# valette/FROG

Hardware: AMD Instinct MI355X
Metric: registration iterations/sec (linear+deformable) (higher is better)
Workload: dtype f32

## Files before the change

frog_amd/_abi.py:

```python
import ctypes as C
import os

_HERE = os.path.dirname(os.path.abspath(__file__))
LIB_DIR = os.path.join(_HERE, "lib")



def usable_cpus():
    import math
    n = len(os.sched_getaffinity(0)) if hasattr(os, "sched_getaffinity") else (os.cpu_count() or 1)

    def quota(d):
        try:
            with open(os.path.join(d, "cpu.max")) as fh:
                q, p = fh.read().split()[:2]
            return None if q == "max" else float(q) / float(p)
        except (OSError, ValueError):
            pass
        try:
            with open(os.path.join(d, "cpu.cfs_quota_us")) as fh:
                q = float(fh.read())
            with open(os.path.join(d, "cpu.cfs_period_us")) as fh:
                p = float(fh.read())
            return q / p if q > 0 and p > 0 else None
# ... 278 lines not shown
    "frog_deformable_phase_b": (C.c_int, [C.c_void_p]),
    "frog_deformable_phase_c": (C.c_int, [C.c_void_p, c_double_p]),
    "frog_get_stream": (C.c_int, [C.c_void_p, C.POINTER(C.c_void_p), C.POINTER(C.c_int)]),
    "frog_comm_unpack_slab": (C.c_int, [C.c_void_p, C.c_void_p, C.c_uint64, C.c_uint32, C.POINTER(C.c_uint64), C.c_uint32]),
    "frog_comm_mode": (C.c_int, [C.c_void_p, C.c_int]),
    "frog_create_seconds": (C.c_int, [C.c_void_p, c_double_p, C.POINTER(C.c_int)]),
    "frog_lattice_reallocations": (C.c_int, [C.c_void_p, C.POINTER(C.c_int)]),
    "frog_transform_points_slab": (C.c_int, [C.c_void_p, C.c_int, C.c_int, C.c_void_p, C.c_uint64, C.c_uint32]),
    "frog_comm_unpack_slab_step": (C.c_int, [C.c_void_p, C.c_void_p, C.c_uint64, C.c_uint32, C.POINTER(C.c_uint64), C.c_uint32, C.c_uint32]),
    "frog_step_finish": (C.c_int, [C.c_void_p, C.POINTER(C.c_double)]),
    "frog_step_speculate": (C.c_int, [C.c_void_p]),
    "frog_cull_stats": (C.c_int, [C.c_void_p, C.POINTER(C.c_uint64), C.POINTER(C.c_uint64), C.POINTER(C.c_uint64)]),
    "frog_cull_stats_linear": (C.c_int, [C.c_void_p, C.POINTER(C.c_uint64), C.POINTER(C.c_uint64), C.POINTER(C.c_uint64)]),
    "frog_test_stray_points": (C.c_int, [C.c_void_p, C.POINTER(C.c_uint64)]),
    "frog_test_cull_ranges": (C.c_int, [C.c_void_p, C.POINTER(C.c_uint64), C.POINTER(C.c_uint64)]),
    "frog_test_em_refit": (C.c_int, [C.c_void_p, C.c_int]),
    "frog_test_inlier_probability": (C.c_int, [C.c_int, c_float_p, c_float_p, C.c_size_t, c_float_p, c_float_p]),
    "frog_test_inlier_weight_pair": (C.c_int, [C.c_int, c_float_p, c_float_p, C.c_float, c_float_p, C.c_size_t, c_float_p,
                                              C.POINTER(C.c_ubyte)]),
    "frog_test_bspline_weights": (C.c_int, [C.c_int, C.c_void_p, C.c_size_t, C.c_void_p]),
    "frog_profile_enable": (C.c_int, [C.c_void_p, C.c_int]),
    "frog_profile_read": (C.c_int, [C.c_void_p, C.POINTER(FrogKernelTime), C.c_int]),
}

HOST_SYMBOLS = {
    "frog_pairs_read": (C.c_void_p, [C.c_char_p, C.POINTER(C.c_int)]),
    "frog_pairs_write": (C.c_int, [C.c_void_p, C.c_char_p]),
    "frog_pairs_free": (None, [C.c_void_p]),
    "frog_pairs_model": (None, [C.c_void_p, C.POINTER(FrogModel)]),
    "frog_pairs_num_pairs": (C.c_uint64, [C.c_void_p]),
# ... 109 lines not shown
```

frog_amd/csrc/device/ctx.h:

```cpp
#pragma once

#include <hip/hip_runtime.h>

#include <cstdint>
#include <cstdio>
#include <cstring>
#include <string>
#include <memory>
#include <vector>

#include "../../../include/frog_hip.h"
#include "dev_buf.h"
#include "switches.h"

namespace frog {

extern thread_local std::string g_last_error;

inline int fail(int code, const std::string &msg)
{
    g_last_error = msg;
    return code;
}

// ... 258 lines not shown
    frog::DevBuf<uint32_t> rc_group_len;
    frog::DevBuf<uint64_t> rc_group_size, rc_group_ptr;
    frog::DevBuf<uint32_t> rc_ent;
    frog::DevBuf<double> rc_wt;

    bool exact_weights = false;
    float fast_theta() const { return sw.weight_general ? __builtin_nanf("") : opt.inlier_threshold - 1e-4f; }
    bool cull_enabled = true;
    bool cull_need_build = true;
    bool cull_linear = true;
    uint64_t cull_lin_builds = 0;
    frog::DevBuf<unsigned long long> lin_listed;
    frog::DevBuf<uint32_t> act_recs32;
    frog::DevBuf<frog::LinkRec> act_recs;
    frog::DevBuf<uint32_t> act_cnt;
    bool pos_b_stale = true;
    frog::DevBuf<float4> pos_b;
    frog::DevBuf<frog::P3> pos2_snap;
    frog::DevBuf<float> cut_now, cut_list;
    frog::DevBuf<uint32_t> disp_part;
    uint32_t disp_n = 0;
    uint32_t disp_own_n = 0;
    bool disp_others = false;
    frog::DevBuf<uint32_t> cull_state;
    frog::DevBuf<float> disp_allow;
    frog::DevBuf<float4> retired_arena;
    size_t retired_used = 0;
    bool coeff_zero = false;
    bool build_in_sweep = false;
    bool cull_check_due = true;
// ... 21 lines not shown
```

frog_amd/csrc/device/frog_hip.hip:

```cpp

#include "ctx.h"
#include <hip/hip_ext.h>
#include "prep.h"
#include "k_links.hip.h"
#include "k_stats.hip.h"
#include "k_grid.hip.h"
#include "k_comm.hip.h"
#include "k_cull.hip.h"
#include "k_ransac.hip.h"
#include "k_reforder.hip.h"
#include "k_refchain.hip.h"
#include "similarity.h"

#include <atomic>
#include <chrono>
#include <cmath>
#include <cstdlib>
#include <random>
#include <limits>
#include <new>

namespace frog {
thread_local std::string g_last_error;
constexpr int BOUNDS_BLOCKS = 256;
// ... 90 lines not shown
}

static SweepArgs sweep_args(frog_ctx *ctx, uint32_t sub)
{
    SweepArgs a;
    a.sub = sub;
    a.n_groups = ctx->n_groups;
    for (uint32_t g = 0; g <= ctx->n_groups; g++) a.group_begin[g] = ctx->group_begin[g];
    a.tiles = ctx->tiles.p; a.recs = ctx->rec_format.narrow ? (const void *)ctx->recs32.p : (const void *)ctx->recs.p; a.pos2 = ctx->pos2.p; a.emd = ctx->emd.p; a.emf = ctx->emf.p; a.em = ctx->em.p;
    a.rec2_last = (uint32_t)(ctx->L_recs / 2 - 1);
    a.img_bits = ctx->rec_format.img_bits; a.lds_images = sweep_lds_images(ctx); a.poff = ctx->d_poff.p; a.point_last = (uint32_t)(ctx->P ? ctx->P - 1 : 0);
    a.n_tiles = ctx->n_tiles; a.threshold = ctx->opt.inlier_threshold;
    a.band = ctx->exact_weights ? __builtin_inff() : THRESHOLD_BAND;
    a.tile_partial = ctx->tile_partial.p; a.tile_counts = ctx->tile_counts.p; a.group_sums = ctx->group_sums.p;
    a.own_pt_begin = ctx->own_pt_begin; a.own_points = ctx->own_pt_end - ctx->own_pt_begin;
    a.act_recs = nullptr; a.act_cnt = nullptr; a.cull_state = nullptr;
    a.cut_list = nullptr; a.build_recs = nullptr; a.build_cnt = nullptr;
    a.point_sums = ctx->point_sums.p; a.tile_order = ctx->tile_order.p; a.tiles_bo = ctx->tiles_bo.p;
    return a;
}

static bool cull_active(const frog_ctx *ctx)
{
    return ctx->cull_enabled && ctx->deformable && ctx->opt.inlier_threshold >= 1e-3f && ctx->n_tiles > 0;
}

static bool cull_active_linear(const frog_ctx *ctx)
{
    return ctx->cull_enabled && ctx->cull_linear && !ctx->exact_weights && !ctx->deformable && ctx->n_tiles > 0 && ctx->n_sub == 1;
}

static bool sweep_builds_list(const frog_ctx *ctx) { return ctx->rec_format.narrow != 0; }
// ... 2 lines not shown
{
    return ctx->fused_sweep && !build;
}

template <int MODE>
static void launch_sweep(frog_ctx *ctx, uint32_t sub, hipStream_t s, hipEvent_t ea = nullptr, hipEvent_t eb = nullptr,
                         bool use_list = false, bool build_list = false)
{
    uint32_t widest = 0;
    for (uint32_t g = 0; g < ctx->n_groups; g++) widest = std::max(widest, ctx->group_begin[g + 1] - ctx->group_begin[g]);
    if (ctx->n_tiles == 0) return;
    SweepArgs args = sweep_args(ctx, sub);
    if (use_list) {
        args.act_recs = ctx->rec_format.narrow ? (const void *)ctx->act_recs32.p : (const void *)ctx->act_recs.p;
        args.act_cnt = ctx->act_cnt.p;
        args.cull_state = ctx->cull_state.p;
    }
    const dim3 grid(sweep_blocks(ctx)), block(256);
    const size_t lds = (size_t)args.lds_images * (sizeof(EmDerived) + sizeof(uint32_t) + sizeof(float));
    if constexpr (MODE == SWEEP_LINEAR) {
        if (build_list && sweep_builds_list(ctx)) {
            args.act_recs = nullptr; args.act_cnt = nullptr;
            args.cut_list = ctx->cut_list.p; args.build_recs = ctx->act_recs32.p; args.build_cnt = ctx->act_cnt.p;
            hipExtLaunchKernelGGL((sweep_kernel<SWEEP_LINEAR, true, false, true>), grid, block, lds, s, ea, eb, 0, args);
            return;
        }
    }
    if constexpr (MODE == SWEEP_DEFORMABLE) {
        const bool build = build_list && sweep_builds_list(ctx);
        if (build) {
            args.act_recs = nullptr; args.act_cnt = nullptr;
            args.cut_list = ctx->cut_list.p; args.build_recs = ctx->act_recs32.p; args.build_cnt = ctx->act_cnt.p;
        }
        if (sweep_fused_now(ctx, build)) {
            const dim3 fgrid(ctx->n_order_blocks), fblock(512);
            const size_t flds = lds * N_XCD;
            if (ctx->rec_format.narrow) hipExtLaunchKernelGGL((sweep_kernel<SWEEP_DEFORMABLE, true, false, false, true>), fgrid, fblock, flds, s, ea, eb, 0, args);
            else hipExtLaunchKernelGGL((sweep_kernel<SWEEP_DEFORMABLE, true, true, false, true>), fgrid, fblock, flds, s, ea, eb, 0, args);
            return;
        }
        if (build) {
            hipExtLaunchKernelGGL((sweep_kernel<SWEEP_DEFORMABLE, true, false, true>), grid, block, lds, s, ea, eb, 0, args);
            return;
        }
    }
    if (ctx->rec_format.narrow)
        hipExtLaunchKernelGGL((sweep_kernel<MODE, true, false>), grid, block, lds, s, ea, eb, 0, args);
// ... 940 lines not shown
    if (o->n_fixed_images) {
        const uint32_t nf = (uint32_t)o->n_fixed_images;
        if (o->n_fixed_images < 0 || nf >= m->n_images) return fail(FROG_E_INVALID, "n_fixed_images must leave at least one moving image");
        if (image_begin != 0 || image_end != m->n_images)
            return fail(FROG_E_INVALID, "n_fixed_images needs the whole group in one context");
        frog_options o2 = *o;
        o2.n_fixed_images = 0;
        frog_ctx *moving = nullptr, *fixed = nullptr;
        int rc = frog_create(m, &o2, device, nf, m->n_images, &moving);
        if (rc) return rc;
        frog_options o3 = o2;
        o3.max_levels_hint = 0;
        rc = frog_create(m, &o3, device, 0, nf, &fixed);
        if (rc) { frog_destroy(moving); return rc; }
        fixed->cull_enabled = false;
        fixed->act_recs32.release(); fixed->act_recs.release(); fixed->act_cnt.release(); fixed->pos2_snap.release();
        rc = frog_set_stream(fixed, moving->stream);
        if (rc) { frog_destroy(fixed); frog_destroy(moving); return rc; }
        moving->helper = fixed;
        moving->nf = nf;
        moving->opt.n_fixed_images = o->n_fixed_images;
        *out = moving;
        return FROG_OK;
    }
    frog_ctx *c = new (std::nothrow) frog_ctx;
    if (!c) return fail(FROG_E_NOMEM, "out of host memory");
    c->sw = read_switches(MAX_SUBPASS);
    c->device = device;
    c->opt = *o;
    c->ib = image_begin; c->ie = image_end;
    if (const int rc = create_stages(c, m)) {
// ... 604 lines not shown
        return fail(FROG_E_STATE, "context owns a sub-range of images: use frog_bounds_local + all-reduce + frog_deformable_setup_bounds");
    double mn[3], mx[3];
    int rc = frog_bounds_local(ctx, mn, mx);
    if (rc) return rc;
    return frog_deformable_setup_bounds(ctx, level, mn, mx, out);
}

static int cull_allocate_buffers(frog_ctx *ctx);

static int cull_allocate(frog_ctx *ctx)
{
    if (ctx->act_cnt.p || !ctx->cull_enabled) return FROG_OK;
    const int rc = cull_allocate_buffers(ctx);
    if (rc == FROG_OK) return rc;
    (void)hipGetLastError();
    ctx->act_recs32.release(); ctx->act_recs.release(); ctx->act_cnt.release(); ctx->pos2_snap.release();
    ctx->cut_list.release(); ctx->disp_part.release(); ctx->cull_state.release(); ctx->disp_allow.release();
    ctx->cull_enabled = false;
    ctx->fused_sweep = ctx->fused_sweep && ctx->sw.fused == 1;
    return FROG_OK;
}

static int cull_allocate_buffers(frog_ctx *ctx)
{
    hipStream_t s = ctx->stream;
    if (ctx->rec_format.narrow) {
        FROG_HIP_CHECK(ctx->act_recs32.alloc(ctx->L_recs));
        FROG_HIP_CHECK(hipMemsetAsync(ctx->act_recs32.p, 0, ctx->act_recs32.bytes(), s));
    } else {
        FROG_HIP_CHECK(ctx->act_recs.alloc(ctx->L_recs));
        FROG_HIP_CHECK(hipMemsetAsync(ctx->act_recs.p, 0, ctx->act_recs.bytes(), s));
    }
    FROG_HIP_CHECK(ctx->act_cnt.alloc(std::max<size_t>(1, (size_t)ctx->n_tiles * ctx->n_groups)));
    FROG_HIP_CHECK(ctx->pos2_snap.alloc(ctx->P));
    FROG_HIP_CHECK(ctx->cut_list.alloc(ctx->nI));
    {
        uint32_t blocks = 0;
        for (uint32_t i = 0; i < ctx->nI; i++) blocks += div_up(ctx->poff[i + 1] - ctx->poff[i], CULL_BLOCK_POINTS);
        FROG_HIP_CHECK(ctx->disp_part.alloc(std::max<size_t>(blocks, (size_t)ctx->P + ctx->P / SCATTER_CHUNK + 16)));
    }
    FROG_HIP_CHECK(ctx->cull_state.alloc(2));
    FROG_HIP_CHECK(hipMemsetAsync(ctx->cull_state.p, 0, ctx->cull_state.bytes(), s));
    FROG_HIP_CHECK(ctx->disp_allow.alloc(1));
    FROG_HIP_CHECK(hipMemsetAsync(ctx->disp_allow.p, 0xFF, sizeof(float), s));
    ctx->cull_need_build = true;
    return FROG_OK;
}

static int cull_prepare(frog_ctx *ctx)
{
    hipStream_t s = ctx->stream;
    const uint32_t nI = ctx->nI;
    int rc = cull_allocate(ctx);
    if (rc) return rc;
    if (!ctx->cull_enabled) return FROG_OK;
    if (ctx->cull_need_build) {
        cull_list_cutoff_kernel<<<div_up(nI, 64), 64, 0, s>>>(ctx->cut_now.p, nI, ctx->deformable ? ctx->sw.cull_scale : ctx->sw.cull_lin_scale,
                                                              ctx->deformable ? ctx->sw.cull_pad : ctx->sw.cull_lin_pad, ctx->cut_list.p);
        FROG_HIP_CHECK(hipMemcpyAsync(ctx->pos2_snap.p, ctx->pos2.p, ctx->P * sizeof(P3), hipMemcpyDeviceToDevice, s));
        ctx->build_in_sweep = sweep_builds_list(ctx) && !ctx->sw.cull_build_pass;
        if (!ctx->build_in_sweep) {
            const SweepArgs args = sweep_args(ctx, 0);
            const dim3 grid(sweep_blocks(ctx), ctx->n_sub);
            if (ctx->rec_format.narrow)
                cull_build_kernel<false><<<grid, 256, 0, s>>>(args, ctx->cut_list.p, ctx->act_recs32.p, ctx->act_cnt.p);
            else
                cull_build_kernel<true><<<grid, 256, 0, s>>>(args, ctx->cut_list.p, ctx->act_recs.p, ctx->act_cnt.p);
            FROG_HIP_CHECK(hipGetLastError());
        }
        ctx->cull_need_build = false;
        if (ctx->deformable) ctx->cull_builds++; else ctx->cull_lin_builds++;
        ctx->disp_n = 0;
        ctx->disp_own_n = 0;
        ctx->disp_current = true;
        ctx->disp_others = true;
        ctx->cull_check_due = true;
    }
    const bool measured = ctx->disp_current && ((ctx->whole_group() && !ctx->xyz2_exported) || ctx->disp_others);
    if (!measured) {
        uint32_t max_pts = 1;
        for (uint32_t i = 0; i < nI; i++) max_pts = std::max(max_pts, ctx->poff[i + 1] - ctx->poff[i]);
        const dim3 grid(div_up(max_pts, CULL_BLOCK_POINTS), nI);
// ... 606 lines not shown
    CTX_GUARD(ctx);
    if (!ranges || !with_election) return fail(FROG_E_INVALID, "null output");
    *ranges = 0; *with_election = 0;
    if (ctx->cull_builds && ctx->act_cnt.n) {
        std::vector<uint32_t> h(ctx->act_cnt.n);
        FROG_HIP_CHECK(hipMemcpyAsync(h.data(), ctx->act_cnt.p, ctx->act_cnt.bytes(), hipMemcpyDeviceToHost, ctx->stream));
        FROG_HIP_CHECK(hipStreamSynchronize(ctx->stream));
        for (uint32_t v : h) {
            if (v & ~CULL_DUP_BIT) (*ranges)++;
            if (v & CULL_DUP_BIT) (*with_election)++;
        }
    }
    return FROG_OK;
}

int frog_test_stray_points(frog_ctx *ctx, uint64_t *n)
{
    CTX_GUARD(ctx);
    { const int rc_ = join_setup(ctx); if (rc_) return rc_; }
    if (!n) return fail(FROG_E_INVALID, "null output");
    unsigned int v = 0;
    FROG_HIP_CHECK(hipMemcpyAsync(&v, ctx->stray.p + 2, sizeof v, hipMemcpyDeviceToHost, ctx->stream));
    FROG_HIP_CHECK(hipStreamSynchronize(ctx->stream));
    *n = v;
    return FROG_OK;
}

int frog_test_em_refit(frog_ctx *ctx, int term_by_term)
{
    CTX_GUARD(ctx);
// ... 199 lines not shown
```

frog_amd/csrc/device/k_cull.hip.h:

```cpp
#pragma once

#include "ctx.h"
#include "k_links.hip.h"
#include "k_stats.hip.h"

namespace frog {

__device__ inline double mixture_probability(double d, double c1, double c2, double ratio)
{
    const double eps = 1e-10, c = 0.797884560802865;
    const double a = d / (c1 + eps), b = d / (c2 + eps);
    const double x1 = ratio * c * a * a * exp(-0.5 * a * a) / (c1 + eps);
    const double x2 = (1.0 - ratio) * c * b * b * exp(-0.5 * b * b) / (c2 + eps);
    return x1 / (x1 + x2 + eps);
}

__device__ inline float cull_cutoff_of(const float4 e, float threshold);

__global__ void cull_cutoff_kernel(const float4 *em, uint32_t n_images, float threshold, float *cut_now)
{
    const uint32_t i = blockIdx.x * blockDim.x + threadIdx.x;
    if (i >= n_images) return;
    cut_now[i] = cull_cutoff_of(em[i], threshold);
}
// ... 43 lines not shown
                out = (float)hi;
            }
        }
        if (out < __builtin_inff()) out = out * 1.000001f + 1e-6f;
    }
    return out;
}

__global__ void cull_list_cutoff_kernel(const float *cut_now, uint32_t n_images, float scale, float pad, float *cut_list)
{
    const uint32_t i = blockIdx.x * blockDim.x + threadIdx.x;
    if (i < n_images) cut_list[i] = scale * cut_now[i] + pad;
}

template <bool WIDE>
__global__ __launch_bounds__(256) void cull_build_kernel(const SweepArgs a, const float *cut_list, void *act_recs, uint32_t *act_cnt)
{
    const int wave = threadIdx.x >> 6, lane = threadIdx.x & 63;
    const uint32_t xcd = blockIdx.x % N_XCD;
    const uint32_t grp = blockIdx.y * N_XCD + xcd;
    const uint32_t t = (blockIdx.x / N_XCD) * 4 + wave;
    if (t >= a.n_tiles) return;
    const Tile &tl = a.tiles[t];
    const uint32_t pt_begin = tl.pt_begin, image = tl.image;
    const uint32_t rec_lo = tl.rec_begin + tl.group_off[grp], rec_n = tl.group_cnt[grp];
    const uint32_t g_first = a.group_begin[grp];
    const float cutA = cut_list[image];
    using Rec = std::conditional_t<WIDE, unsigned long long, unsigned int>;
    const Rec *src = reinterpret_cast<const Rec *>(a.recs);
    Rec *dst = reinterpret_cast<Rec *>(act_recs);
    auto phys = [&](uint32_t k) { return (size_t)rec_lo + (k / REC_CHUNK) * REC_CHUNK + (k % 64u) * 2u + (k % REC_CHUNK) / 64u; };
    __shared__ uint32_t last_step_s[4][TILE_POINTS];
    uint32_t *last_step = last_step_s[wave];
    for (int k = lane; k < TILE_POINTS; k += 64) last_step[k] = 0xFFFFFFFFu;
    __builtin_amdgcn_fence(__ATOMIC_RELEASE, "wavefront");
    __builtin_amdgcn_wave_barrier();
    bool dup = false;
    uint32_t base = 0;
    constexpr int UNROLL = 4;
    for (uint32_t k0 = 0; k0 < rec_n; k0 += 64 * UNROLL) {
        Rec rq[UNROLL];
        bool have[UNROLL];
        #pragma unroll
        for (int u = 0; u < UNROLL; u++) {
            const uint32_t k = k0 + 64 * u + lane;
            have[u] = k < rec_n;
            rq[u] = have[u] ? src[phys(k)] : (Rec)0;
        }
        P3 pa[UNROLL], pb[UNROLL];
        uint32_t imgB[UNROLL];
        #pragma unroll
        for (int u = 0; u < UNROLL; u++) {
// ... 4 lines not shown
                pb_index = (uint32_t)(rq[u] >> 32);
            } else {
                imgB[u] = g_first + __builtin_amdgcn_ubfe((uint32_t)rq[u], 8u, a.img_bits);
                pb_index = a.poff[imgB[u]] + ((uint32_t)rq[u] >> (8u + a.img_bits));
            }
            pa[u] = a.pos2[pt_begin + ia];
            pb[u] = a.pos2[min(pb_index, a.point_last)];
        }
        #pragma unroll
        for (int u = 0; u < UNROLL; u++) {
            const float dx = pb[u].x - pa[u].x, dy = pb[u].y - pa[u].y, dz = pb[u].z - pa[u].z;
            const float d2 = dx * dx + dy * dy + dz * dz;
            const float cut = have[u] ? fminf(cutA, cut_list[imgB[u]]) : 0.f;
            const bool keep = have[u] && !(d2 >= cut * cut);
            const unsigned long long m = __ballot(keep);
            if (keep) {
                const uint32_t to = base + (uint32_t)__popcll(m & ((1ull << lane) - 1ull));
                dst[phys(to)] = rq[u];
                dup |= atomicExch(&last_step[(uint32_t)rq[u] & 0xFFu], to >> 6) == (to >> 6);
            }
            base += (uint32_t)__popcll(m);
        }
    }
    const bool any_dup = __ballot(dup) != 0ull;
    if (lane == 0) act_cnt[(size_t)t * a.n_groups + grp] = base | (any_dup ? CULL_DUP_BIT : 0u);
    const uint32_t cap = (rec_n + REC_CHUNK - 1) / REC_CHUNK * REC_CHUNK;
    const uint32_t reach = (((base + 63u) / 64u + BODY_STEPS - 1u) / BODY_STEPS * BODY_STEPS + PT_AHEAD) * 64u;
    for (uint32_t k = base + lane; k < min(cap, reach); k += 64) dst[phys(k)] = (Rec)0;
}

constexpr int CULL_BLOCK_POINTS = 2048;

__global__ __launch_bounds__(256) void cull_disp_kernel(const P3 *pos2, const P3 *snap, const uint32_t *poff, uint32_t *disp_part)
{
    __shared__ uint32_t sh[4];
    const uint32_t img = blockIdx.y;
    const uint32_t p0 = poff[img] + blockIdx.x * CULL_BLOCK_POINTS, pe = poff[img + 1];
    const uint32_t p1 = min(p0 + (uint32_t)CULL_BLOCK_POINTS, pe);
    uint32_t m = 0;
// ... 117 lines not shown
```

frog_amd/csrc/device/k_links.hip.h:

```cpp
#pragma once

#include "ctx.h"

#include <type_traits>

namespace frog {

enum { SWEEP_LINEAR = 0, SWEEP_DEFORMABLE = 1, SWEEP_COUNT = 2 };
constexpr int CHUNK_RING = 3, CHUNK_AHEAD = 2;
constexpr int PT_RING = 3, PT_AHEAD = 2;
constexpr int BODY_STEPS = 6;
static_assert(BODY_STEPS == 2 * CHUNK_RING && BODY_STEPS % PT_RING == 0 && PT_AHEAD < PT_RING && CHUNK_AHEAD < CHUNK_RING
              && 2 * CHUNK_AHEAD >= PT_AHEAD + 2, "ring periods must divide the unrolled body; a gather needs its record");
constexpr int EMD_LDS_IMAGES = 256;
constexpr uint32_t CULL_DUP_BIT = 0x80000000u;
constexpr int OWNER_WORDS = TILE_POINTS / 2;
static_assert((OWNER_WORDS & (OWNER_WORDS - 1)) == 0, "the election word of a point is its index masked");
static_assert(EMD_LDS_IMAGES == 1 << 8, "prep.h admits narrow records for img_bits <= 8 only");
constexpr int LINEAR_SUMS = 18;

struct SweepArgs {
    const Tile *tiles;
    const void *recs;
    const uint32_t *poff;
    uint32_t img_bits;
    uint32_t lds_images;
    uint32_t point_last;
    const P3 *pos2;
    const EmDerived *emd;
    const EmFast *emf;
// ... 2 lines not shown
    uint32_t rec2_last;
    float threshold;
    float band;
    double *tile_partial;
    long long *tile_counts;
    float4 *group_sums;
    float4 *point_sums;
    const uint32_t *tile_order;
    const Tile *tiles_bo;
    uint32_t own_pt_begin, own_points;
    uint32_t sub;
    uint32_t n_groups;
    uint32_t group_begin[MAX_GROUPS + 1];
    const void *act_recs;
    const uint32_t *act_cnt;
    const uint32_t *cull_state;
    const float *cut_list;
    void *build_recs;
    uint32_t *build_cnt;
};


__device__ __forceinline__ float sqrt_rn(float x)
{
    const float s = __builtin_amdgcn_sqrtf(x);
    const float lo = __uint_as_float(__float_as_uint(s) - 1u), hi = __uint_as_float(__float_as_uint(s) + 1u);
    const float e_lo = __builtin_fmaf(-lo, s, x), e_hi = __builtin_fmaf(-hi, s, x);
    float r = (0.0f >= e_lo) ? lo : s;
    r = (0.0f < e_hi) ? hi : r;
    return r;
}

__device__ __forceinline__ float div_fast(float n, float d)
{
// ... 22 lines not shown
constexpr float INLIER_PROBABILITY_BOUND = 1.52587890625e-05f;
constexpr float D2_FIX = __builtin_bit_cast(float, 0x3c23d70au);
__device__ __forceinline__ float inlier_probability(float d2, const EmDerived e)
{
    const float e1 = __builtin_amdgcn_exp2f(d2 * e.s1), e2 = __builtin_amdgcn_exp2f(d2 * e.s2);
    const float x1 = e.kq1 * (d2 * e1), x2 = e.kq2 * (d2 * e2);
    const float p = div_fast(x1, x1 + x2 + 1e-10f);
    return d2 < D2_FIX ? 1.0f : p;
}

__device__ __forceinline__ float inlier_weight_pair(float d2, const EmFast a, const EmFast b, bool &in_range)
{
    const float e = fmaxf(__builtin_fmaf(a.ds, d2, a.l), __builtin_fmaf(b.ds, d2, b.l));
    in_range = d2 >= b.lo && d2 <= b.hi;
    return __builtin_amdgcn_rcpf(1.0f + __builtin_amdgcn_exp2f(e));
}

__device__ __forceinline__ double wave_sum(double v)
{
    #pragma unroll
    for (int off = 32; off > 0; off >>= 1) v += __shfl_down(v, off, 64);
    return v;
}

__device__ __forceinline__ long long wave_sum_ll(long long v)
{
    #pragma unroll
    for (int off = 32; off > 0; off >>= 1) v += __shfl_down(v, off, 64);
    return v;
}
// ... 32 lines not shown
    const uint32_t xcd = FUSED ? (uint32_t)wave : blockIdx.x % N_XCD;
    const uint32_t grp = FUSED ? (uint32_t)wave : a.sub * N_XCD + xcd;
    const uint32_t t = FUSED ? a.tile_order[blockIdx.x] : (blockIdx.x / N_XCD) * 4 + wave;
    const bool live = t < a.n_tiles;

    uint32_t pt_begin = 0, pt_count = 0, rec_lo = 0, rec_n = 0, image = 0;
    if (FUSED || live) {
        const Tile &tl = FUSED ? a.tiles_bo[blockIdx.x] : a.tiles[t];
        pt_begin = tl.pt_begin; pt_count = tl.pt_count; image = tl.image;
        rec_lo = tl.rec_begin + tl.group_off[grp];
        rec_n = tl.group_cnt[grp];
    }
    bool listed = false;
    if constexpr (MODE != SWEEP_COUNT) listed = a.act_cnt != nullptr && a.cull_state[0] == 0u;
    bool elect = true;
    if (listed && live) {
        const uint32_t c = a.act_cnt[(size_t)t * a.n_groups + grp];
        rec_n = c & ~CULL_DUP_BIT;
        elect = (c & CULL_DUP_BIT) != 0u;
    }
    elect = __builtin_amdgcn_readfirstlane((uint32_t)elect) != 0u;
    rec_lo = __builtin_amdgcn_readfirstlane(rec_lo);
    rec_n = __builtin_amdgcn_readfirstlane(rec_n);
    pt_begin = __builtin_amdgcn_readfirstlane(pt_begin);
    pt_count = __builtin_amdgcn_readfirstlane(pt_count);
    image = __builtin_amdgcn_readfirstlane(image);
    float4 *my = acc + (MODE == SWEEP_DEFORMABLE ? wave * TILE_POINTS : 0);
    unsigned int *own = owner + (MODE == SWEEP_DEFORMABLE ? wave * OWNER_WORDS : 0);

    if (MODE == SWEEP_DEFORMABLE) {
        for (int k = lane; k < TILE_POINTS; k += 64) {
            my[k] = (a.sub > 0 && (uint32_t)k < pt_count) ? a.group_sums[group_sum_index(xcd, pt_begin - a.own_pt_begin + k, a.own_points)]
                                                          : make_float4(0.f, 0.f, 0.f, 0.f);
            if (k < OWNER_WORDS) own[k] = 0xFFFFFFFFu;
        }
    }
    typedef unsigned long long v2u64 __attribute__((ext_vector_type(2)));
    typedef unsigned int v2u32 __attribute__((ext_vector_type(2)));
    using Rec = std::conditional_t<WIDE, unsigned long long, unsigned int>;
    using Chunk = std::conditional_t<WIDE, v2u64, v2u32>;
    const Chunk *rec2 = reinterpret_cast<const Chunk *>(listed ? a.act_recs : a.recs);
// ... 30 lines not shown
        }
        else { for (uint32_t k = fill_id; k < g_count; k += fill_stride) emd_s[k] = a.emd[g_first + k]; }
    }
    if (!WIDE)
        for (uint32_t k = fill_id; k < a.lds_images; k += fill_stride) img_base_s[k] = k < g_count ? a.poff[g_first + k] : 0u;
    uint32_t *last_step = last_step_s + (BUILD ? wave * TILE_POINTS : 0);
    if constexpr (BUILD) {
        for (uint32_t k = fill_id; k < a.lds_images; k += fill_stride) cut_s[k] = k < g_count ? a.cut_list[g_first + k] : 0.f;
        for (int k = lane; k < TILE_POINTS; k += 64) last_step[k] = 0xFFFFFFFFu;
    }
    __syncthreads();
    FROG_TR(2);
    const float cutA = BUILD ? a.cut_list[image] : 0.f;
    uint32_t built = 0;
    bool dup = false;

    const EmDerived eA = a.emd[image];
    const EmFast fA = a.emf[image];

    double s[(MODE == SWEEP_LINEAR) ? LINEAR_SUMS : 2];
    #pragma unroll
    for (int k = 0; k < ((MODE == SWEEP_LINEAR) ? LINEAR_SUMS : 2); k++) s[k] = 0.0;
    long long n_in = 0, n_out = 0;

    const uint32_t img_bits = a.img_bits;
    auto own_of = [&](Rec rq) { return (uint32_t)rq & 0xFFu; };
    auto img_of = [&](Rec rq) {
        if constexpr (WIDE) return ((uint32_t)rq >> 8) - (EMD_LDS ? g_first : 0u);
        else return __builtin_amdgcn_ubfe((uint32_t)rq, 8u, img_bits);
    };
    auto gather = [&](Rec rq) {
        if constexpr (WIDE) return a.pos2[(uint32_t)(rq >> 32)];
        else return a.pos2[min(img_base_s[img_of(rq)] + ((uint32_t)rq >> (8u + img_bits)), a.point_last)];
    };
    Chunk cq[CHUNK_RING];
    P3 pbq[PT_RING];
    #pragma unroll
    for (int k = 0; k < CHUNK_RING; k++) cq[k] = (k < CHUNK_AHEAD) ? cq_first[k < CHUNK_AHEAD ? k : 0] : Chunk{ 0, 0 };
    #pragma unroll
    for (int k = 0; k < PT_RING; k++) pbq[k] = (k < PT_AHEAD) ? gather((k & 1) ? cq[k / 2].y : cq[k / 2].x) : P3{ 0.f, 0.f, 0.f };

    auto step = [&](const Rec rq, const P3 pb, auto elect_c, const bool valid) __attribute__((always_inline)) {
        constexpr bool ELECT = decltype(elect_c)::value;
        const uint32_t ia = own_of(rq);
        const P3 pa = { px[ia], px[ia + PLANE], px[ia + 2 * PLANE] };
        EmDerived eB;
        EmFast fB;
        if constexpr (W1) {
            fB = EMD_LDS ? emf_s[img_of(rq)] : a.emf[img_of(rq)];
            if constexpr (!(EMD_LDS && FUSED)) { fB.lo = fmaxf(fB.lo, fA.lo); fB.hi = fminf(fB.hi, fA.hi); }
        }
        else eB = EMD_LDS ? emd_s[img_of(rq)] : a.emd[img_of(rq)];

        const float dx = pb.x - pa.x, dy = pb.y - pa.y, dz = pb.z - pa.z;
        const float d2 = dx * dx + dy * dy + dz * dz;
        if constexpr (BUILD) {
            const float cut = fminf(cutA, cut_s[img_of(rq)]);
            const bool keep = valid && !(d2 >= cut * cut);
            const unsigned long long m = __ballot(keep);
            if (keep) {
                const uint32_t to = built + (uint32_t)__popcll(m & ((1ull << lane) - 1ull));
                reinterpret_cast<Rec *>(a.build_recs)[(size_t)rec_lo + (to / REC_CHUNK) * REC_CHUNK + (to % 64u) * 2u + (to % REC_CHUNK) / 64u] = rq;
                dup |= atomicExch(&last_step[ia], to >> 6) == (to >> 6);
            }
            built += (uint32_t)__popcll(m);
            if (!valid) return;
        }
        float w;
        if constexpr (W1) {
            bool in_range;
            w = inlier_weight_pair(d2, fA, fB, in_range);
            asm volatile("" : "+v"(w));
            if (!in_range && !(w < a.threshold - a.band)) {
                const uint32_t imgB = img_of(rq) + (WIDE && !EMD_LDS ? 0u : g_first);
                w = fminf(inlier_probability(d2, eA), inlier_probability(d2, a.emd[imgB]));
            }
        } else w = fminf(inlier_probability(d2, eA), inlier_probability(d2, eB));
        if constexpr (MODE != SWEEP_LINEAR) {
            if (fabsf(w - a.threshold) < a.band) {
// ... 10 lines not shown
        if constexpr (MODE == SWEEP_LINEAR) {
            const float d = sqrt_rn(d2);
            s[16] += (double)(w * w * d * d);
            s[17] += (double)(w * w);
            s[0] += (double)(w * dx); s[1] += (double)(w * dy); s[2] += (double)(w * dz);
            s[3] += (double)(w * pa.x); s[4] += (double)(w * pa.y); s[5] += (double)(w * pa.z);
            s[6] += (double)(w * pb.x); s[7] += (double)(w * pb.y); s[8] += (double)(w * pb.z);
            s[9] += (double)(w * pa.x * pa.x); s[10] += (double)(w * pa.y * pa.y); s[11] += (double)(w * pa.z * pa.z);
            s[12] += (double)(w * pb.x * pb.x); s[13] += (double)(w * pb.y * pb.y); s[14] += (double)(w * pb.z * pb.z);
            s[15] += (double)w;
        } else if constexpr (MODE == SWEEP_DEFORMABLE) {
            const bool inlier = w >= a.threshold;
            const float w2 = w * w;
            s[1] += (double)(inlier ? w2 : 0.0f);
            s[0] += (double)(inlier ? w2 * d2 : 0.0f);
            if constexpr (!ELECT) {
                if (inlier) {
                    float4 t = my[ia];
                    t.x += w2 * dx; t.y += w2 * dy; t.z += w2 * dz; t.w += w2;
                    my[ia] = t;
                }
                __builtin_amdgcn_fence(__ATOMIC_RELEASE, "wavefront");
                __builtin_amdgcn_wave_barrier();
                return;
            }
            bool pending = inlier;
            const uint32_t io = ia & (OWNER_WORDS - 1);
            while (__ballot(pending)) {
                if (pending) atomicMin(&own[io], (unsigned int)lane);
                __builtin_amdgcn_fence(__ATOMIC_RELEASE, "wavefront");
                __builtin_amdgcn_wave_barrier();
// ... 3 lines not shown
                    my[ia] = t;
                    own[io] = 0xFFFFFFFFu;
                    pending = false;
                }
                __builtin_amdgcn_fence(__ATOMIC_RELEASE, "wavefront");
                __builtin_amdgcn_wave_barrier();
            }
        } else {
            if (w < a.threshold) n_out++; else n_in++;
        }
    };

    const uint32_t n_steps = (rec_n + 63) / 64;
    auto walk = [&](auto elect_c) __attribute__((always_inline)) {
        for (uint32_t base = 0; base < n_steps; base += BODY_STEPS) {
            #pragma unroll
            for (int j = 0; j < BODY_STEPS; j++) {
                const uint32_t r = lane + 64 * (base + j);
                if (j % 2 == 0) cq[(j / 2 + CHUNK_AHEAD) % CHUNK_RING] = chunk_at(base / 2 + j / 2 + CHUNK_AHEAD);
                {
                    const Chunk ahead = cq[((j + PT_AHEAD) / 2) % CHUNK_RING];
                    pbq[(j + PT_AHEAD) % PT_RING] = gather(((j + PT_AHEAD) & 1) ? ahead.y : ahead.x);
                }
                if (BUILD || r < rec_n) step((j & 1) ? cq[j / 2].y : cq[j / 2].x, pbq[j % PT_RING], elect_c, r < rec_n);
#ifdef FROG_SWEEP_TRACE
                if (base == 0 && j == 0) FROG_TR(3);
#endif
            }
        }
    };
    if (MODE != SWEEP_DEFORMABLE || elect) walk(std::true_type{});
    else walk(std::false_type{});
    FROG_TR(4);

    if constexpr (BUILD) {
        const uint32_t cap = (rec_n + REC_CHUNK - 1) / REC_CHUNK * REC_CHUNK;
        const uint32_t reach = (((built + 63u) / 64u + BODY_STEPS - 1u) / BODY_STEPS * BODY_STEPS + PT_AHEAD) * 64u;
        for (uint32_t k = built + lane; k < min(cap, reach); k += 64)
            reinterpret_cast<Rec *>(a.build_recs)[(size_t)rec_lo + (k / REC_CHUNK) * REC_CHUNK + (k % 64u) * 2u + (k % REC_CHUNK) / 64u] = (Rec)0;
    }
    if constexpr (MODE == SWEEP_LINEAR) {
        #pragma unroll
        for (int k = 0; k < LINEAR_SUMS; k++) {
            double v = wave_sum(s[k]);
            if (lane == 0 && live) a.tile_partial[((size_t)t * a.n_groups + grp) * LINEAR_SUMS + k] = v;
        }
        if constexpr (BUILD) {
            if (lane == 0 && live) a.build_cnt[(size_t)t * a.n_groups + grp] = built | CULL_DUP_BIT;
        }
    } else if constexpr (MODE == SWEEP_DEFORMABLE) {
        double v0 = wave_sum(s[0]), v1 = wave_sum(s[1]);
        if (lane == 0 && live) {
            a.tile_partial[((size_t)t * a.n_groups + grp) * 2] = v0;
            a.tile_partial[((size_t)t * a.n_groups + grp) * 2 + 1] = v1;
        }
        if constexpr (BUILD) {
            const bool any_dup = __ballot(dup) != 0ull;
            if (lane == 0 && live) a.build_cnt[(size_t)t * a.n_groups + grp] = built | (any_dup ? CULL_DUP_BIT : 0u);
        }
        __syncthreads();
        FROG_TR(5);
        typedef float v4f __attribute__((ext_vector_type(4)));
        if constexpr (FUSED) {
            for (uint32_t k = threadIdx.x; k < pt_count; k += 64 * WAVES) {
                float4 v = acc[k];
                #pragma unroll
                for (int g = 1; g < N_XCD; g++) {
                    const float4 u = acc[g * TILE_POINTS + k];
                    v.x += u.x; v.y += u.y; v.z += u.z; v.w += u.w;
                }
                a.point_sums[pt_begin + k] = v;
            }
// ... 197 lines not shown
```

frog_amd/image_group.py:

```python
import ctypes as C

import numpy as np

from . import _abi, schedule
from ._abi import check


class ImageGroup:
    def __init__(self, pairs=None, device=0, image_range=None, **options):
        self.linearIterations = 50
        self.deformableLevels = 3
        self.deformableIterations = 200
        self.deformableAlpha = 0.02
        self.linearInitializationAnchor = (0.5, 0.5, 0.5)
        self.statIntervalUpdate = 10
        self.opt = _abi.FrogOptions.default()
        for k, v in options.items():
            if hasattr(self.opt, k):
                setattr(self.opt, k, v)
            elif hasattr(self, k):
                setattr(self, k, v)
            else:
                raise AttributeError(k)
        self._lib = _abi.hip_lib()
# ... 192 lines not shown
    def cull_stats_linear(self):
        a, b, c = C.c_uint64(), C.c_uint64(), C.c_uint64()
        check(self._lib.frog_cull_stats_linear(self._ctx, C.byref(a), C.byref(b), C.byref(c)), "frog_cull_stats_linear")
        return a.value, b.value, c.value

    def cull_stats(self):
        a, b, c = C.c_uint64(), C.c_uint64(), C.c_uint64()
        check(self._lib.frog_cull_stats(self._ctx, C.byref(a), C.byref(b), C.byref(c)), "frog_cull_stats")
        return a.value, b.value, c.value

    def cull_ranges(self):
        a, b = C.c_uint64(), C.c_uint64()
        check(self._lib.frog_test_cull_ranges(self._ctx, C.byref(a), C.byref(b)), "frog_test_cull_ranges")
        return a.value, b.value

    def stray_points(self):
        n = C.c_uint64()
        check(self._lib.frog_test_stray_points(self._ctx, C.byref(n)), "frog_test_stray_points")
        return n.value

    def residualSums(self):
        check(self._lib.frog_residual_sums(self._ctx), "frog_residual_sums")

    def gradient(self, image, n_cp):
        out = np.empty((n_cp, 4), np.float32)
        check(self._lib.frog_get_gradient(self._ctx, image, out.ctypes.data_as(_abi.c_float_p), 4 * n_cp),
              "frog_get_gradient")
        return out


# ... 24 lines not shown
```

include/frog_hip.h:

```cpp
#ifndef FROG_HIP_H
#define FROG_HIP_H

#include "frog_types.h"

#ifdef __cplusplus
extern "C" {
#endif

typedef struct frog_ctx frog_ctx;


int frog_device_count(void);
int frog_device_warm(int device);
const char *frog_last_error(void);

int frog_create(const frog_model *model, const frog_options *options, int device,
                uint32_t image_begin, uint32_t image_end, frog_ctx **out);
void frog_destroy(frog_ctx *ctx);

int frog_set_stream(frog_ctx *ctx, void *hip_stream);
int frog_create_seconds(frog_ctx *ctx, double seconds3[3], int *selections_replayed);
int frog_lattice_reallocations(frog_ctx *ctx, int *count);

int frog_get_stream(frog_ctx *ctx, void **hip_stream, int *device);
// ... 76 lines not shown
int frog_deformable_phase_c(frog_ctx *ctx, double *E);

int frog_cull_stats(frog_ctx *ctx, uint64_t *lists_built, uint64_t *listed_half_links, uint64_t *owned_half_links);
int frog_cull_stats_linear(frog_ctx *ctx, uint64_t *lists_built, uint64_t *listed_half_links, uint64_t *owned_half_links);

int frog_test_inlier_probability(int device, const float c1_c2_ratio[3], const float *d2, size_t n,
                                 float *fast, float *exact);

int frog_test_inlier_weight_pair(int device, const float c1_c2_ratio_a[3], const float c1_c2_ratio_b[3], float inlier_threshold,
                                 const float *d2, size_t n, float *weight, unsigned char *form);

int frog_test_bspline_weights(int device, const double *f, size_t n, double *out4n);

int frog_test_stray_points(frog_ctx *ctx, uint64_t *n);
int frog_test_cull_ranges(frog_ctx *ctx, uint64_t *ranges, uint64_t *with_election);

int frog_test_em_refit(frog_ctx *ctx, int term_by_term);

enum {
    FROG_K_SWEEP_LINEAR = 0,
    FROG_K_SWEEP_DEFORMABLE,
    FROG_K_SCATTER,
    FROG_K_LATTICE,
    FROG_K_TRANSFORM,
    FROG_K_STATS,
    FROG_K_COMBINE,
    FROG_K_CULL,
    FROG_K_SWEEP_BUILD,
    FROG_K_SWEEP_LINEAR_BUILD,
    FROG_K_COUNT_
// ... 13 lines not shown
```

Baseline: 2383.

## Track duplicate-owner elections per 64-record step in culled deformable sweeps

When the cull list is built, a bitmap now records which 64-record steps hold two links sharing the same owner point in the same step. The deformable sweep then takes the atomic election path only on those flagged steps within a 64-step window and accumulates the rest directly into LDS, instead of electing across a whole tile once any duplicate is present. This is meant to cut atomic and election overhead in the deformable sweep. The cost is extra ballots and atomicOr in the build kernels, loads of the step words at sweep start, and more code variants that may raise register pressure.

Measured after the change: 2483, median of 6. +4.2%, better.

```diff
diff --git a/frog_amd/_abi.py b/frog_amd/_abi.py
--- a/frog_amd/_abi.py
+++ b/frog_amd/_abi.py
@@ -316,6 +316,7 @@
     "frog_cull_stats_linear": (C.c_int, [C.c_void_p, C.POINTER(C.c_uint64), C.POINTER(C.c_uint64), C.POINTER(C.c_uint64)]),
     "frog_test_stray_points": (C.c_int, [C.c_void_p, C.POINTER(C.c_uint64)]),
     "frog_test_cull_ranges": (C.c_int, [C.c_void_p, C.POINTER(C.c_uint64), C.POINTER(C.c_uint64)]),
+    "frog_test_cull_steps": (C.c_int, [C.c_void_p, C.POINTER(C.c_uint64), C.POINTER(C.c_uint64)]),
     "frog_test_em_refit": (C.c_int, [C.c_void_p, C.c_int]),
     "frog_test_inlier_probability": (C.c_int, [C.c_int, c_float_p, c_float_p, C.c_size_t, c_float_p, c_float_p]),
     "frog_test_inlier_weight_pair": (C.c_int, [C.c_int, c_float_p, c_float_p, C.c_float, c_float_p, C.c_size_t, c_float_p,
diff --git a/frog_amd/csrc/device/ctx.h b/frog_amd/csrc/device/ctx.h
--- a/frog_amd/csrc/device/ctx.h
+++ b/frog_amd/csrc/device/ctx.h
@@ -296,6 +296,7 @@
     frog::DevBuf<uint32_t> act_recs32;
     frog::DevBuf<frog::LinkRec> act_recs;
     frog::DevBuf<uint32_t> act_cnt;
+    frog::DevBuf<uint32_t> act_steps;
     bool pos_b_stale = true;
     frog::DevBuf<float4> pos_b;
     frog::DevBuf<frog::P3> pos2_snap;
diff --git a/frog_amd/csrc/device/frog_hip.hip b/frog_amd/csrc/device/frog_hip.hip
--- a/frog_amd/csrc/device/frog_hip.hip
+++ b/frog_amd/csrc/device/frog_hip.hip
@@ -128,8 +128,8 @@
     a.band = ctx->exact_weights ? __builtin_inff() : THRESHOLD_BAND;
     a.tile_partial = ctx->tile_partial.p; a.tile_counts = ctx->tile_counts.p; a.group_sums = ctx->group_sums.p;
     a.own_pt_begin = ctx->own_pt_begin; a.own_points = ctx->own_pt_end - ctx->own_pt_begin;
-    a.act_recs = nullptr; a.act_cnt = nullptr; a.cull_state = nullptr;
-    a.cut_list = nullptr; a.build_recs = nullptr; a.build_cnt = nullptr;
+    a.act_recs = nullptr; a.act_cnt = nullptr; a.act_steps = nullptr; a.cull_state = nullptr;
+    a.cut_list = nullptr; a.build_recs = nullptr; a.build_cnt = nullptr; a.build_steps = nullptr;
     a.point_sums = ctx->point_sums.p; a.tile_order = ctx->tile_order.p; a.tiles_bo = ctx->tiles_bo.p;
     return a;
 }
@@ -162,6 +162,7 @@
     if (use_list) {
         args.act_recs = ctx->rec_format.narrow ? (const void *)ctx->act_recs32.p : (const void *)ctx->act_recs.p;
         args.act_cnt = ctx->act_cnt.p;
+        args.act_steps = ctx->act_steps.p;
         args.cull_state = ctx->cull_state.p;
     }
     const dim3 grid(sweep_blocks(ctx)), block(256);
@@ -179,6 +180,7 @@
         if (build) {
             args.act_recs = nullptr; args.act_cnt = nullptr;
             args.cut_list = ctx->cut_list.p; args.build_recs = ctx->act_recs32.p; args.build_cnt = ctx->act_cnt.p;
+            args.build_steps = ctx->act_steps.p;
         }
         if (sweep_fused_now(ctx, build)) {
             const dim3 fgrid(ctx->n_order_blocks), fblock(512);
@@ -1149,7 +1151,7 @@
         rc = frog_create(m, &o3, device, 0, nf, &fixed);
         if (rc) { frog_destroy(moving); return rc; }
         fixed->cull_enabled = false;
-        fixed->act_recs32.release(); fixed->act_recs.release(); fixed->act_cnt.release(); fixed->pos2_snap.release();
+        fixed->act_recs32.release(); fixed->act_recs.release(); fixed->act_cnt.release(); fixed->act_steps.release(); fixed->pos2_snap.release();
         rc = frog_set_stream(fixed, moving->stream);
         if (rc) { frog_destroy(fixed); frog_destroy(moving); return rc; }
         moving->helper = fixed;
@@ -1784,12 +1786,14 @@
     const int rc = cull_allocate_buffers(ctx);
     if (rc == FROG_OK) return rc;
     (void)hipGetLastError();
-    ctx->act_recs32.release(); ctx->act_recs.release(); ctx->act_cnt.release(); ctx->pos2_snap.release();
+    ctx->act_recs32.release(); ctx->act_recs.release(); ctx->act_cnt.release(); ctx->act_steps.release(); ctx->pos2_snap.release();
     ctx->cut_list.release(); ctx->disp_part.release(); ctx->cull_state.release(); ctx->disp_allow.release();
     ctx->cull_enabled = false;
     ctx->fused_sweep = ctx->fused_sweep && ctx->sw.fused == 1;
     return FROG_OK;
 }
+
+static size_t cull_step_words(const frog_ctx *ctx) { return (size_t)((ctx->L_recs / 64 + 31) / 32); }
 
 static int cull_allocate_buffers(frog_ctx *ctx)
 {
@@ -1802,6 +1806,8 @@
         FROG_HIP_CHECK(hipMemsetAsync(ctx->act_recs.p, 0, ctx->act_recs.bytes(), s));
     }
     FROG_HIP_CHECK(ctx->act_cnt.alloc(std::max<size_t>(1, (size_t)ctx->n_tiles * ctx->n_groups)));
+    FROG_HIP_CHECK(ctx->act_steps.alloc(cull_step_words(ctx) + 2));
+    FROG_HIP_CHECK(hipMemsetAsync(ctx->act_steps.p, 0, ctx->act_steps.bytes(), s));
     FROG_HIP_CHECK(ctx->pos2_snap.alloc(ctx->P));
     FROG_HIP_CHECK(ctx->cut_list.alloc(ctx->nI));
     {
@@ -1829,13 +1835,15 @@
                                                               ctx->deformable ? ctx->sw.cull_pad : ctx->sw.cull_lin_pad, ctx->cut_list.p);
         FROG_HIP_CHECK(hipMemcpyAsync(ctx->pos2_snap.p, ctx->pos2.p, ctx->P * sizeof(P3), hipMemcpyDeviceToDevice, s));
         ctx->build_in_sweep = sweep_builds_list(ctx) && !ctx->sw.cull_build_pass;
+        FROG_HIP_CHECK(hipMemsetAsync(ctx->act_steps.p, 0, ctx->act_steps.bytes(), s));
+        uint32_t *steps = ctx->deformable ? ctx->act_steps.p : nullptr;
         if (!ctx->build_in_sweep) {
             const SweepArgs args = sweep_args(ctx, 0);
             const dim3 grid(sweep_blocks(ctx), ctx->n_sub);
             if (ctx->rec_format.narrow)
-                cull_build_kernel<false><<<grid, 256, 0, s>>>(args, ctx->cut_list.p, ctx->act_recs32.p, ctx->act_cnt.p);
+                cull_build_kernel<false><<<grid, 256, 0, s>>>(args, ctx->cut_list.p, ctx->act_recs32.p, ctx->act_cnt.p, steps);
             else
-                cull_build_kernel<true><<<grid, 256, 0, s>>>(args, ctx->cut_list.p, ctx->act_recs.p, ctx->act_cnt.p);
+                cull_build_kernel<true><<<grid, 256, 0, s>>>(args, ctx->cut_list.p, ctx->act_recs.p, ctx->act_cnt.p, steps);
             FROG_HIP_CHECK(hipGetLastError());
         }
         ctx->cull_need_build = false;
@@ -2472,6 +2480,22 @@
     return FROG_OK;
 }
 
+int frog_test_cull_steps(frog_ctx *ctx, uint64_t *listed_steps, uint64_t *steps_with_election)
+{
+    CTX_GUARD(ctx);
+    if (!listed_steps || !steps_with_election) return fail(FROG_E_INVALID, "null output");
+    *listed_steps = 0; *steps_with_election = 0;
+    if (ctx->cull_builds && ctx->act_cnt.n) {
+        std::vector<uint32_t> h(ctx->act_cnt.n), bits(ctx->act_steps.n);
+        FROG_HIP_CHECK(hipMemcpyAsync(h.data(), ctx->act_cnt.p, ctx->act_cnt.bytes(), hipMemcpyDeviceToHost, ctx->stream));
+        FROG_HIP_CHECK(hipMemcpyAsync(bits.data(), ctx->act_steps.p, ctx->act_steps.bytes(), hipMemcpyDeviceToHost, ctx->stream));
+        FROG_HIP_CHECK(hipStreamSynchronize(ctx->stream));
+        for (uint32_t v : h) *listed_steps += ((v & ~CULL_DUP_BIT) + 63u) / 64u;
+        for (uint32_t v : bits) *steps_with_election += (uint64_t)__builtin_popcount(v);
+    }
+    return FROG_OK;
+}
+
 int frog_test_stray_points(frog_ctx *ctx, uint64_t *n)
 {
     CTX_GUARD(ctx);
diff --git a/frog_amd/csrc/device/k_cull.hip.h b/frog_amd/csrc/device/k_cull.hip.h
--- a/frog_amd/csrc/device/k_cull.hip.h
+++ b/frog_amd/csrc/device/k_cull.hip.h
@@ -81,7 +81,8 @@
 }
 
 template <bool WIDE>
-__global__ __launch_bounds__(256) void cull_build_kernel(const SweepArgs a, const float *cut_list, void *act_recs, uint32_t *act_cnt)
+__global__ __launch_bounds__(256) void cull_build_kernel(const SweepArgs a, const float *cut_list, void *act_recs, uint32_t *act_cnt,
+                                                         uint32_t *act_steps)
 {
     const int wave = threadIdx.x >> 6, lane = threadIdx.x & 63;
     const uint32_t xcd = blockIdx.x % N_XCD;
@@ -103,6 +104,7 @@
     __builtin_amdgcn_fence(__ATOMIC_RELEASE, "wavefront");
     __builtin_amdgcn_wave_barrier();
     bool dup = false;
+    DupSteps dup_steps;
     uint32_t base = 0;
     constexpr int UNROLL = 4;
     for (uint32_t k0 = 0; k0 < rec_n; k0 += 64 * UNROLL) {
@@ -137,15 +139,19 @@
             const float cut = have[u] ? fminf(cutA, cut_list[imgB[u]]) : 0.f;
             const bool keep = have[u] && !(d2 >= cut * cut);
             const unsigned long long m = __ballot(keep);
+            const uint32_t to = base + (uint32_t)__popcll(m & ((1ull << lane) - 1ull));
+            bool hit = false;
             if (keep) {
-                const uint32_t to = base + (uint32_t)__popcll(m & ((1ull << lane) - 1ull));
                 dst[phys(to)] = rq[u];
-                dup |= atomicExch(&last_step[(uint32_t)rq[u] & 0xFFu], to >> 6) == (to >> 6);
-            }
+                hit = atomicExch(&last_step[(uint32_t)rq[u] & 0xFFu], to >> 6) == (to >> 6);
+            }
+            dup |= hit;
+            if (act_steps) dup_steps_add(act_steps, dup_steps, rec_lo >> 6, hit, to, base, lane);
             base += (uint32_t)__popcll(m);
         }
     }
     const bool any_dup = __ballot(dup) != 0ull;
+    if (act_steps) dup_steps_flush(act_steps, dup_steps, lane);
     if (lane == 0) act_cnt[(size_t)t * a.n_groups + grp] = base | (any_dup ? CULL_DUP_BIT : 0u);
     const uint32_t cap = (rec_n + REC_CHUNK - 1) / REC_CHUNK * REC_CHUNK;
     const uint32_t reach = (((base + 63u) / 64u + BODY_STEPS - 1u) / BODY_STEPS * BODY_STEPS + PT_AHEAD) * 64u;
diff --git a/frog_amd/csrc/device/k_links.hip.h b/frog_amd/csrc/device/k_links.hip.h
--- a/frog_amd/csrc/device/k_links.hip.h
+++ b/frog_amd/csrc/device/k_links.hip.h
@@ -14,6 +14,7 @@
               && 2 * CHUNK_AHEAD >= PT_AHEAD + 2, "ring periods must divide the unrolled body; a gather needs its record");
 constexpr int EMD_LDS_IMAGES = 256;
 constexpr uint32_t CULL_DUP_BIT = 0x80000000u;
+constexpr int STEP_WINDOW = 64;
 constexpr int OWNER_WORDS = TILE_POINTS / 2;
 static_assert((OWNER_WORDS & (OWNER_WORDS - 1)) == 0, "the election word of a point is its index masked");
 static_assert(EMD_LDS_IMAGES == 1 << 8, "prep.h admits narrow records for img_bits <= 8 only");
@@ -46,10 +47,12 @@
     uint32_t group_begin[MAX_GROUPS + 1];
     const void *act_recs;
     const uint32_t *act_cnt;
+    const uint32_t *act_steps;
     const uint32_t *cull_state;
     const float *cut_list;
     void *build_recs;
     uint32_t *build_cnt;
+    uint32_t *build_steps;
 };
 
 
@@ -102,6 +105,24 @@
     const float e = fmaxf(__builtin_fmaf(a.ds, d2, a.l), __builtin_fmaf(b.ds, d2, b.l));
     in_range = d2 >= b.lo && d2 <= b.hi;
     return __builtin_amdgcn_rcpf(1.0f + __builtin_amdgcn_exp2f(e));
+}
+
+struct DupSteps { uint32_t word = 0xFFFFFFFFu, bits = 0u; };
+__device__ __forceinline__ void dup_steps_flush(uint32_t *steps, const DupSteps &d, int lane)
+{
+    if (d.bits != 0u && lane == 0) atomicOr(&steps[d.word], d.bits);
+}
+__device__ __forceinline__ void dup_steps_mark(uint32_t *steps, DupSteps &d, uint32_t bit, int lane)
+{
+    if ((bit >> 5) != d.word) { dup_steps_flush(steps, d, lane); d.word = bit >> 5; d.bits = 0u; }
+    d.bits |= 1u << (bit & 31u);
+}
+__device__ __forceinline__ void dup_steps_add(uint32_t *steps, DupSteps &d, uint32_t bit0, bool hit, uint32_t to, uint32_t built, int lane)
+{
+    if (__ballot(hit) == 0ull) return;
+    const uint32_t s0 = built >> 6;
+    if (__ballot(hit && (to >> 6) == s0) != 0ull) dup_steps_mark(steps, d, bit0 + s0, lane);
+    if (__ballot(hit && (to >> 6) != s0) != 0ull) dup_steps_mark(steps, d, bit0 + s0 + 1u, lane);
 }
 
 __device__ __forceinline__ double wave_sum(double v)
@@ -164,17 +185,31 @@
     bool listed = false;
     if constexpr (MODE != SWEEP_COUNT) listed = a.act_cnt != nullptr && a.cull_state[0] == 0u;
     bool elect = true;
+    bool by_step = false;
+    uint32_t sw[3] = { 0u, 0u, 0u };
     if (listed && live) {
+        if constexpr (MODE == SWEEP_DEFORMABLE) {
+            const uint32_t *w = a.act_steps + (rec_lo >> 11);
+            sw[0] = w[0]; sw[1] = w[1]; sw[2] = w[2];
+            __builtin_amdgcn_sched_barrier(0);
+        }
         const uint32_t c = a.act_cnt[(size_t)t * a.n_groups + grp];
         rec_n = c & ~CULL_DUP_BIT;
         elect = (c & CULL_DUP_BIT) != 0u;
+        by_step = elect && MODE == SWEEP_DEFORMABLE;
     }
     elect = __builtin_amdgcn_readfirstlane((uint32_t)elect) != 0u;
+    by_step = __builtin_amdgcn_readfirstlane((uint32_t)by_step) != 0u;
     rec_lo = __builtin_amdgcn_readfirstlane(rec_lo);
     rec_n = __builtin_amdgcn_readfirstlane(rec_n);
     pt_begin = __builtin_amdgcn_readfirstlane(pt_begin);
     pt_count = __builtin_amdgcn_readfirstlane(pt_count);
     image = __builtin_amdgcn_readfirstlane(image);
+    const uint32_t win_sh = (rec_lo >> 6) & 31u;
+    const uint32_t win_lo = __builtin_amdgcn_readfirstlane((uint32_t)((((unsigned long long)sw[1] << 32) | sw[0]) >> win_sh));
+    const uint32_t win_hi = __builtin_amdgcn_readfirstlane((uint32_t)((((unsigned long long)sw[2] << 32) | sw[1]) >> win_sh));
+    const unsigned long long win = ((unsigned long long)win_hi << 32) | win_lo;
+    static_assert(STEP_WINDOW == 64, "the window is one 64-bit scalar");
     float4 *my = acc + (MODE == SWEEP_DEFORMABLE ? wave * TILE_POINTS : 0);
     unsigned int *own = owner + (MODE == SWEEP_DEFORMABLE ? wave * OWNER_WORDS : 0);
 
@@ -235,6 +270,7 @@
     const float cutA = BUILD ? a.cut_list[image] : 0.f;
     uint32_t built = 0;
     bool dup = false;
+    DupSteps dup_steps;
 
     const EmDerived eA = a.emd[image];
     const EmFast fA = a.emf[image];
@@ -261,8 +297,8 @@
     #pragma unroll
     for (int k = 0; k < PT_RING; k++) pbq[k] = (k < PT_AHEAD) ? gather((k & 1) ? cq[k / 2].y : cq[k / 2].x) : P3{ 0.f, 0.f, 0.f };
 
-    auto step = [&](const Rec rq, const P3 pb, auto elect_c, const bool valid) __attribute__((always_inline)) {
-        constexpr bool ELECT = decltype(elect_c)::value;
+    auto step = [&](const Rec rq, const P3 pb, auto elect_c, const bool elect_now, const bool valid) __attribute__((always_inline)) {
+        constexpr int ELECT = decltype(elect_c)::value;
         const uint32_t ia = own_of(rq);
         const P3 pa = { px[ia], px[ia + PLANE], px[ia + 2 * PLANE] };
         EmDerived eB;
@@ -279,11 +315,14 @@
             const float cut = fminf(cutA, cut_s[img_of(rq)]);
             const bool keep = valid && !(d2 >= cut * cut);
             const unsigned long long m = __ballot(keep);
+            const uint32_t to = built + (uint32_t)__popcll(m & ((1ull << lane) - 1ull));
+            bool hit = false;
             if (keep) {
-                const uint32_t to = built + (uint32_t)__popcll(m & ((1ull << lane) - 1ull));
                 reinterpret_cast<Rec *>(a.build_recs)[(size_t)rec_lo + (to / REC_CHUNK) * REC_CHUNK + (to % 64u) * 2u + (to % REC_CHUNK) / 64u] = rq;
-                dup |= atomicExch(&last_step[ia], to >> 6) == (to >> 6);
-            }
+                hit = atomicExch(&last_step[ia], to >> 6) == (to >> 6);
+            }
+            dup |= hit;
+            if constexpr (MODE == SWEEP_DEFORMABLE) dup_steps_add(a.build_steps, dup_steps, rec_lo >> 6, hit, to, built, lane);
             built += (uint32_t)__popcll(m);
             if (!valid) return;
         }
@@ -324,7 +363,7 @@
             const float w2 = w * w;
             s[1] += (double)(inlier ? w2 : 0.0f);
             s[0] += (double)(inlier ? w2 * d2 : 0.0f);
-            if constexpr (!ELECT) {
+            if (ELECT == 0 || (ELECT == 2 && !elect_now)) {
                 if (inlier) {
                     float4 t = my[ia];
                     t.x += w2 * dx; t.y += w2 * dy; t.z += w2 * dz; t.w += w2;
@@ -358,6 +397,8 @@
     const uint32_t n_steps = (rec_n + 63) / 64;
     auto walk = [&](auto elect_c) __attribute__((always_inline)) {
         for (uint32_t base = 0; base < n_steps; base += BODY_STEPS) {
+            uint32_t trip = 0u;
+            if constexpr (decltype(elect_c)::value == 2) trip = base < (uint32_t)STEP_WINDOW ? ~(uint32_t)(~win >> base) : ~0u;
             #pragma unroll
             for (int j = 0; j < BODY_STEPS; j++) {
                 const uint32_t r = lane + 64 * (base + j);
@@ -366,15 +407,16 @@
                     const Chunk ahead = cq[((j + PT_AHEAD) / 2) % CHUNK_RING];
                     pbq[(j + PT_AHEAD) % PT_RING] = gather(((j + PT_AHEAD) & 1) ? ahead.y : ahead.x);
                 }
-                if (BUILD || r < rec_n) step((j & 1) ? cq[j / 2].y : cq[j / 2].x, pbq[j % PT_RING], elect_c, r < rec_n);
+                if (BUILD || r < rec_n) step((j & 1) ? cq[j / 2].y : cq[j / 2].x, pbq[j % PT_RING], elect_c, (trip >> j & 1u) != 0u, r < rec_n);
 #ifdef FROG_SWEEP_TRACE
                 if (base == 0 && j == 0) FROG_TR(3);
 #endif
             }
         }
     };
-    if (MODE != SWEEP_DEFORMABLE || elect) walk(std::true_type{});
-    else walk(std::false_type{});
+    if (MODE == SWEEP_DEFORMABLE && !elect) walk(std::integral_constant<int, 0>{});
+    else if (MODE == SWEEP_DEFORMABLE && by_step) walk(std::integral_constant<int, 2>{});
+    else walk(std::integral_constant<int, 1>{});
     FROG_TR(4);
 
     if constexpr (BUILD) {
@@ -400,6 +442,7 @@
         }
         if constexpr (BUILD) {
             const bool any_dup = __ballot(dup) != 0ull;
+            dup_steps_flush(a.build_steps, dup_steps, lane);
             if (lane == 0 && live) a.build_cnt[(size_t)t * a.n_groups + grp] = built | (any_dup ? CULL_DUP_BIT : 0u);
         }
         __syncthreads();
diff --git a/frog_amd/image_group.py b/frog_amd/image_group.py
--- a/frog_amd/image_group.py
+++ b/frog_amd/image_group.py
@@ -230,6 +230,11 @@
         check(self._lib.frog_test_cull_ranges(self._ctx, C.byref(a), C.byref(b)), "frog_test_cull_ranges")
         return a.value, b.value
 
+    def cull_steps(self):
+        a, b = C.c_uint64(), C.c_uint64()
+        check(self._lib.frog_test_cull_steps(self._ctx, C.byref(a), C.byref(b)), "frog_test_cull_steps")
+        return a.value, b.value
+
     def stray_points(self):
         n = C.c_uint64()
         check(self._lib.frog_test_stray_points(self._ctx, C.byref(n)), "frog_test_stray_points")
diff --git a/include/frog_hip.h b/include/frog_hip.h
--- a/include/frog_hip.h
+++ b/include/frog_hip.h
@@ -114,6 +114,7 @@
 
 int frog_test_stray_points(frog_ctx *ctx, uint64_t *n);
 int frog_test_cull_ranges(frog_ctx *ctx, uint64_t *ranges, uint64_t *with_election);
+int frog_test_cull_steps(frog_ctx *ctx, uint64_t *listed_steps, uint64_t *steps_with_election);
 
 int frog_test_em_refit(frog_ctx *ctx, int term_by_term);
 
```
